# UVA-Computer-Vision-Lab/FrameINO

Hardware: AMD Instinct MI355X
Metric: denoise-steps/sec (Wan2.2-5B FrameINO, 49f 704x1280, cond+uncond DiT forward + CFG + Euler) (higher is better)
Workload: dtype bf16; 1 GPU; wan2.2-5b-49f-704x1280; layers=30, id_frames=1, hip_graph=False, parallelism=single, dead_rows_last_block=1760

## Files before the change

### frameino_amd/csrc/fino_elementwise.hip

```cpp
#include <type_traits>

#include "fino_common.h"
#include "fino_gemm_common.h"

namespace {

constexpr int kWavesPerBlock = 4;
constexpr int kMaxPasses = 8;

template <typename T, int NP>
struct RowRegs {
    float v[NP][8];
};

#ifndef FINO_EW_NT
#define FINO_EW_NT 0
#endif
#define EW_STORE_NT(PTR_, VAL_)                                                                \
    {                                                                                          \
        const uint4 v__ = (VAL_);                                                              \
        __builtin_nontemporal_store(u32x4_t{v__.x, v__.y, v__.z, v__.w}, reinterpret_cast<u32x4_t*>(PTR_)); \
    }
#define EW_STORE(PTR_, VAL_) (*reinterpret_cast<uint4*>(PTR_) = (VAL_))

template <typename T, int NP, bool NT = false>
__device__ __forceinline__ void load_row(const uint16_t* __restrict__ p, int dim, int lane, float (&v)[NP][8]) {
#pragma unroll
    for (int i = 0; i < NP; ++i) {
        const int c = (i * 64 + lane) * 8;
        if (c < dim) {
            uint4 u;
            if constexpr (NT) {
                const u32x4_t t4 = __builtin_nontemporal_load(reinterpret_cast<const u32x4_t*>(p + c));
                u = make_uint4(t4[0], t4[1], t4[2], t4[3]);
            } else {
                u = *reinterpret_cast<const uint4*>(p + c);
            }
            unpack8<T>(u, v[i]);
        } else {
#pragma unroll
            for (int j = 0; j < 8; ++j) v[i][j] = 0.f;
        }
    }
}

template <int NP>
__device__ __forceinline__ void ln_stats(const float (&v)[NP][8], int dim, int lane, float eps, float& mean,
                                         float& rstd) {
    float s = 0.f;
#pragma unroll
    for (int i = 0; i < NP; ++i)
#pragma unroll
        for (int j = 0; j < 8; ++j) s += v[i][j];
    mean = wave_sum(s) / (float)dim;
    float q = 0.f;
#pragma unroll
    for (int i = 0; i < NP; ++i) {
        const int c = (i * 64 + lane) * 8;
        if (c < dim) {
#pragma unroll
            for (int j = 0; j < 8; ++j) {
                const float d = v[i][j] - mean;
                q += d * d;
            }
        }
    }
    const float var = wave_sum(q) / (float)dim;
    rstd = 1.0f / sqrtf(var + eps);
}

template <typename T, int NP, int MODE, bool QOUT = false>
__global__ __launch_bounds__(kWavesPerBlock * 64) void ln_modulate_kernel(
    const uint16_t* __restrict__ x, uint16_t* __restrict__ y, int64_t rows, int dim, int64_t ldx, int64_t ldy,
    const float* __restrict__ p_w, const float* __restrict__ p_b, const float* __restrict__ p_shift,
    const float* __restrict__ p_scale, int64_t mod_stride, const int32_t* __restrict__ sel, float eps,
    uint8_t* __restrict__ q = nullptr, uint8_t* __restrict__ qs = nullptr, int64_t rows_pad = 0) {
    const int lane = threadIdx.x & 63;
    const int64_t row = (int64_t)blockIdx.x * kWavesPerBlock + (threadIdx.x >> 6);
    if (row >= rows) return;
    float v[NP][8];
    load_row<T, NP, (FINO_EW_NT & 1) != 0>(x + row * ldx, dim, lane, v);
    float mean, rstd;
    ln_stats<NP>(v, dim, lane, eps, mean, rstd);
    const int64_t moff = (MODE != 1 && sel) ? (int64_t)sel[row] * mod_stride : 0;
    auto ld8 = [](const float* p, float (&o)[8]) {
        const float4 a0 = *reinterpret_cast<const float4*>(p);
        const float4 a1 = *reinterpret_cast<const float4*>(p + 4);
        o[0] = a0.x; o[1] = a0.y; o[2] = a0.z; o[3] = a0.w; o[4] = a1.x; o[5] = a1.y; o[6] = a1.z; o[7] = a1.w;
    };
#pragma unroll
    for (int i = 0; i < NP; ++i) {
        const int c = (i * 64 + lane) * 8;
        if (c >= dim) continue;
        float o[8], w[8], b[8], sc[8], sh[8];
        if (MODE != 0 && p_w) ld8(p_w + c, w);
        if (MODE != 0 && p_b) ld8(p_b + c, b);
        if (MODE != 1) { ld8(p_scale + moff + c, sc); ld8(p_shift + moff + c, sh); }
#pragma unroll
        for (int j = 0; j < 8; ++j) {
            const float n = (v[i][j] - mean) * rstd;
            if (MODE == 0) {
                o[j] = n * (1.0f + sc[j]) + sh[j];
            } else {
                float t = n;
                if (p_w) t = t * w[j];
                if (p_b) t = t + b[j];
                if (MODE == 2) t = round_to<T>(round_to<T>(t) * round_to<T>(1.0f + sc[j])) + sh[j];
                o[j] = t;
            }
        }
        if constexpr (QOUT) {
            float r8[8];
#pragma unroll
            for (int j = 0; j < 8; ++j) r8[j] = round_to<T>(o[j]);
            int e;
            const uint2 qv = fino_gemm_ns::mx_quant8(r8, e);
            *reinterpret_cast<uint2*>(q + row * dim + c) = qv;
            if ((c & 31) == 0) qs[fino_gemm_ns::mx_scale_index(row, c, rows_pad)] = (uint8_t)(e + 127);
        } else if constexpr ((FINO_EW_NT & 2) != 0) EW_STORE_NT(y + row * ldy + c, pack8<T>(o))
        else EW_STORE(y + row * ldy + c, pack8<T>(o));
    }
}

template <typename T>
__global__ __launch_bounds__(256) void gated_residual_kernel(const uint16_t* __restrict__ x,
                                                             const uint16_t* __restrict__ y,
                                                             uint16_t* __restrict__ out, int64_t rows, int dim,
                                                             int64_t ldx, int64_t ldy, int64_t ldo,
                                                             const float* __restrict__ gate, int64_t mod_stride,
                                                             const int32_t* __restrict__ sel, int staged) {
    const int chunks = dim >> 3;
    const int64_t total = rows * chunks;
    for (int64_t i = (int64_t)blockIdx.x * blockDim.x + threadIdx.x; i < total;
         i += (int64_t)gridDim.x * blockDim.x) {
        const int64_t row = i / chunks;
        const int c = (int)(i - row * chunks) * 8;
        float a[8], b[8], o[8];
        unpack8<T>(*reinterpret_cast<const uint4*>(x + row * ldx + c), a);
        unpack8<T>(*reinterpret_cast<const uint4*>(y + row * ldy + c), b);
        if (gate) {
            const float* g = gate + (sel ? (int64_t)sel[row] * mod_stride : 0) + c;
            const float4 g0 = *reinterpret_cast<const float4*>(g);
            const float4 g1 = *reinterpret_cast<const float4*>(g + 4);
            const float gg[8] = {g0.x, g0.y, g0.z, g0.w, g1.x, g1.y, g1.z, g1.w};
#pragma unroll
            for (int j = 0; j < 8; ++j) o[j] = a[j] + (staged ? round_to<T>(b[j] * gg[j]) : b[j] * gg[j]);
        } else {
#pragma unroll
            for (int j = 0; j < 8; ++j) o[j] = a[j] + b[j];
        }
        *reinterpret_cast<uint4*>(out + row * ldo + c) = pack8<T>(o);
    }
}

template <typename T, int NP>
__device__ __forceinline__ void rmsnorm_rope_row(uint16_t* __restrict__ xrow, int64_t row, int dim,
                                                 const uint16_t* __restrict__ w, float eps,
                                                 const float* __restrict__ cos_t, const float* __restrict__ sin_t,
                                                 int head_dim, float out_scale, uint16_t* __restrict__ out,
                                                 const int64_t* __restrict__ head_off,
                                                 const int64_t* __restrict__ head_ld, int lane) {
    float v[NP][8];
    load_row<T, NP>(xrow, dim, lane, v);
    float rs = 1.f;
    if (w) {
        float q = 0.f;
#pragma unroll
        for (int i = 0; i < NP; ++i)
#pragma unroll
            for (int j = 0; j < 8; ++j) q += v[i][j] * v[i][j];
        const float var = wave_sum(q) / (float)dim;
        rs = 1.0f / sqrtf(var + eps);
    }
    const int half = head_dim >> 1;
#pragma unroll
    for (int i = 0; i < NP; ++i) {
        const int c = (i * 64 + lane) * 8;
        if (c >= dim) continue;
        float o[8];
        if (w) {
            float ww[8];
            unpack8<T>(*reinterpret_cast<const uint4*>(w + c), ww);
#pragma unroll
            for (int j = 0; j < 8; ++j) o[j] = round_to<T>(round_to<T>(v[i][j] * rs) * ww[j]);
        } else {
#pragma unroll
            for (int j = 0; j < 8; ++j) o[j] = v[i][j];
        }
        if (cos_t) {
            const int pidx = (c % head_dim) >> 1;
            const float4 cs = *reinterpret_cast<const float4*>(cos_t + row * half + pidx);
            const float4 sn = *reinterpret_cast<const float4*>(sin_t + row * half + pidx);
            const float cc[4] = {cs.x, cs.y, cs.z, cs.w};
            const float ss[4] = {sn.x, sn.y, sn.z, sn.w};
#pragma unroll
            for (int j = 0; j < 4; ++j) {
                const float x1 = o[2 * j], x2 = o[2 * j + 1];
                o[2 * j] = x1 * cc[j] - x2 * ss[j];
                o[2 * j + 1] = x1 * ss[j] + x2 * cc[j];
            }
        }
#pragma unroll
        for (int j = 0; j < 8; ++j) o[j] *= out_scale;
        if (out) {
            const int hd = c / head_dim;
            EW_STORE(out + head_off[hd] + row * head_ld[hd] + (c - hd * head_dim), pack8<T>(o));
        } else {
            EW_STORE(xrow + c, pack8<T>(o));
        }
    }
}

struct RmsRopeParts {
    const uint16_t* w[3];
    float eps[3];
    float out_scale[3];
    int rope[3];
};
template <typename T, int NP>
__global__ __launch_bounds__(kWavesPerBlock * 64) void rmsnorm_rope_kernel(uint16_t* __restrict__ x, int64_t rows,
                                                                           int dim, int64_t ldx, const RmsRopeParts pp,
                                                                           const float* __restrict__ cos_t,
                                                                           const float* __restrict__ sin_t,
                                                                           int head_dim, uint16_t* __restrict__ out,
                                                                           const int64_t* __restrict__ head_off,
                                                                           const int64_t* __restrict__ head_ld) {
    const int lane = threadIdx.x & 63;
    const int64_t row = (int64_t)blockIdx.x * kWavesPerBlock + (threadIdx.x >> 6);
    if (row >= rows) return;
    const int s = blockIdx.y;
    const bool rope = pp.rope[s] != 0;
    rmsnorm_rope_row<T, NP>(x + row * ldx + (int64_t)s * dim, row, dim, pp.w[s], pp.eps[s], rope ? cos_t : nullptr,
                            rope ? sin_t : nullptr, head_dim, pp.out_scale[s], out,
                            head_off ? head_off + (int64_t)s * (dim / head_dim) : nullptr, head_ld, lane);
}

template <typename T, int NP>
__global__ __launch_bounds__(kWavesPerBlock * 64) void row_rrms_kernel(const uint16_t* __restrict__ x, int64_t rows, int dim,
                                                                       int64_t ldx, float eps, float* __restrict__ rrms) {
    const int lane = threadIdx.x & 63;
    const int64_t row = (int64_t)blockIdx.x * kWavesPerBlock + (threadIdx.x >> 6);
    if (row >= rows) return;
    float v[NP][8];
    load_row<T, NP>(x + row * ldx, dim, lane, v);
    float q = 0.f;
#pragma unroll
    for (int i = 0; i < NP; ++i)
#pragma unroll
        for (int j = 0; j < 8; ++j) q += v[i][j] * v[i][j];
    const float var = wave_sum(q) / (float)dim;
    if (lane == 0) rrms[row] = 1.0f / sqrtf(var + eps);
}

template <typename T>
__global__ __launch_bounds__(256) void headnorm_rope_kernel(uint16_t* __restrict__ x, int batch, int64_t rows,
                                                            int heads, int head_dim, int64_t ldx,
                                                            int64_t batch_stride, const uint16_t* __restrict__ w,
                                                            const uint16_t* __restrict__ b, float eps,
                                                            const float* __restrict__ cos_t,
                                                            const float* __restrict__ sin_t, int64_t rope_row0,
                                                            float out_scale) {
    const int lanes_per_head = head_dim >> 3;
    const int64_t chunks_per_row = (int64_t)heads * lanes_per_head;
    const int64_t total = (int64_t)batch * rows * chunks_per_row;
    const int64_t i = (int64_t)blockIdx.x * blockDim.x + threadIdx.x;
    const bool active = i < total;
    const int64_t ii = active ? i : total - 1;
    const int64_t br = ii / chunks_per_row;
    const int cw = (int)(ii - br * chunks_per_row);
    const int64_t bi = br / rows;
    const int64_t row = br - bi * rows;
    const int cin = (cw % lanes_per_head) * 8;
    uint16_t* p = x + bi * batch_stride + row * ldx + (int64_t)cw * 8;
    float v[8];
    unpack8<T>(*reinterpret_cast<const uint4*>(p), v);
    if (w) {
        float s = 0.f;
#pragma unroll
        for (int j = 0; j < 8; ++j) s += v[j];
        for (int off = lanes_per_head >> 1; off > 0; off >>= 1) s += __shfl_xor(s, off, 64);
        const float mean = s / (float)head_dim;
        float q = 0.f;
#pragma unroll
        for (int j = 0; j < 8; ++j) {
            const float d = v[j] - mean;
            q += d * d;
        }
        for (int off = lanes_per_head >> 1; off > 0; off >>= 1) q += __shfl_xor(q, off, 64);
        const float rstd = 1.0f / sqrtf(q / (float)head_dim + eps);
        float ww[8], bb[8];
        unpack8<T>(*reinterpret_cast<const uint4*>(w + cin), ww);
        unpack8<T>(*reinterpret_cast<const uint4*>(b + cin), bb);
#pragma unroll
        for (int j = 0; j < 8; ++j) v[j] = round_to<T>((v[j] - mean) * rstd * ww[j] + bb[j]);
    }
    if (cos_t && row >= rope_row0) {
        const float* cp = cos_t + (row - rope_row0) * head_dim + cin;
        const float* sp = sin_t + (row - rope_row0) * head_dim + cin;
        float cc[8], ss[8];
        *reinterpret_cast<float4*>(cc) = *reinterpret_cast<const float4*>(cp);
        *reinterpret_cast<float4*>(cc + 4) = *reinterpret_cast<const float4*>(cp + 4);
        *reinterpret_cast<float4*>(ss) = *reinterpret_cast<const float4*>(sp);
        *reinterpret_cast<float4*>(ss + 4) = *reinterpret_cast<const float4*>(sp + 4);
        float o[8];
#pragma unroll
        for (int j = 0; j < 4; ++j) {
            const float xr = v[2 * j], xi = v[2 * j + 1];
            o[2 * j] = xr * cc[2 * j] + (-xi) * ss[2 * j];
            o[2 * j + 1] = xi * cc[2 * j + 1] + xr * ss[2 * j + 1];
        }
#pragma unroll
        for (int j = 0; j < 8; ++j) v[j] = o[j];
    }
#pragma unroll
    for (int j = 0; j < 8; ++j) v[j] *= out_scale;
    if (active) *reinterpret_cast<uint4*>(p) = pack8<T>(v);
}
// ... 120 lines not shown
    const float sa = coef[0], sb = coef[1], m1 = coef[2], m2 = coef[3], m3 = coef[4], m4 = coef[5], mn = coef[6];
    const float g = coef[7];
    const bool use_old = coef[8] != 0.f;
    for (int64_t i = (int64_t)blockIdx.x * blockDim.x + threadIdx.x; i < n_lat; i += (int64_t)gridDim.x * blockDim.x) {
        float v;
        if (has_uncond) {
            const float u = T::to_f32(pred[i]);
            const float c = T::to_f32(pred[batch_stride + i]);
            v = u + g * (c - u);
        } else {
            v = T::to_f32(pred[i]);
        }
        const float x = T::to_f32(lat[i]);
        const float x0 = round_to<T>(sa * x) - sb * v;
        const float d = use_old ? m3 * x0 - m4 * x0_old[i] : x0;
        const float nz = round_to<T>(mn * T::to_f32(noise[i]));
        lat[i] = T::from_f32(round_to<T>(m1 * x) - m2 * d + nz);
        x0_old[i] = x0;
    }
}

template <typename T>
__device__ __forceinline__ float round_product(float a, float b) {
    if constexpr (std::is_same<T, F16>::value) {
        uint32_t r = 0;
        asm("v_fma_mixlo_f16 %0, %1, %2, 0" : "+v"(r) : "v"(a), "v"(b));
        return F16::to_f32((uint16_t)r);
    } else {
        return round_to<T>(a * b);
    }
}

template <typename T>
__global__ __launch_bounds__(256) void cfg_unipc_kernel(const uint16_t* __restrict__ pc, const uint16_t* __restrict__ pu,
                                                        float* __restrict__ x, float* __restrict__ last,
                                                        float* __restrict__ m0, float* __restrict__ m1, int C, int Fg,
                                                        int Ft, int HW, const float* __restrict__ coef) {
    const float g = coef[0], sigma = coef[1], use_corr = coef[2];
    const float Cx = coef[3], C0 = coef[4], C1 = coef[5], Ct = coef[6], Px = coef[7], P0 = coef[8], P1 = coef[9];
    const int64_t total = (int64_t)C * Fg * HW;
    for (int64_t i = (int64_t)blockIdx.x * blockDim.x + threadIdx.x; i < total;
         i += (int64_t)gridDim.x * blockDim.x) {
        const int s = (int)(i % HW);
        const int f = (int)((i / HW) % Fg);
        const int c = (int)(i / ((int64_t)HW * Fg));
        const int64_t pi = ((int64_t)c * Ft + f) * HW + s;
        float v = T::to_f32(pc[pi]);
        if (pu) {
            const float u = T::to_f32(pu[pi]);
            v = round_to<T>(u + round_to<T>(g * round_to<T>(v - u)));
        }
        const float xv = x[i], a0 = m0[i];
        const float mt = xv - round_product<T>(sigma, v);
        const float xc = use_corr != 0.f ? Cx * last[i] + C0 * a0 + C1 * m1[i] + Ct * mt : xv;
        x[i] = Px * xc + P0 * mt + P1 * a0;
        last[i] = xc;
        m1[i] = a0;
        m0[i] = mt;
    }
}

template <int NPmax, typename F>
inline bool dispatch_np(int dim, F&& f) {
    const int np = (dim + 511) / 512;
    switch (np) {
        case 1: f(std::integral_constant<int, 1>{}); return true;
        case 2: f(std::integral_constant<int, 2>{}); return true;
        case 3: f(std::integral_constant<int, 3>{}); return true;
        case 4: f(std::integral_constant<int, 4>{}); return true;
        case 5: f(std::integral_constant<int, 5>{}); return true;
        case 6: f(std::integral_constant<int, 6>{}); return true;
        case 7: f(std::integral_constant<int, 7>{}); return true;
        case 8: f(std::integral_constant<int, 8>{}); return true;
        default: return false;
    }
}

inline int grid_1d(int64_t total, int block = 256) {
    int64_t g = (total + block - 1) / block;
    const int64_t cap = 256 * 8;
    return (int)(g < 1 ? 1 : (g > cap ? cap : g));
}

template <int MODE>
int launch_ln_q(const void* x, void* q, void* qs, int64_t rows, int dim, int64_t ldx, const float* w, const float* b,
                const float* shift, const float* scale, int64_t mod_stride, const int32_t* sel, float eps, int dtype,
                hipStream_t st) {
    const dim3 grid((unsigned)((rows + kWavesPerBlock - 1) / kWavesPerBlock)), block(kWavesPerBlock * 64);
    const int64_t rows_pad = (rows + 255) / 256 * 256;
    const bool ok = dispatch_np<kMaxPasses>(dim, [&](auto np) {
        constexpr int NP = decltype(np)::value;
        if (dtype == FINO_BF16)
            ln_modulate_kernel<BF16, NP, MODE, true><<<grid, block, 0, st>>>((const uint16_t*)x, nullptr, rows, dim, ldx, 0, w,
                                                                           b, shift, scale, mod_stride, sel, eps,
                                                                           (uint8_t*)q, (uint8_t*)qs, rows_pad);
        else
            ln_modulate_kernel<F16, NP, MODE, true><<<grid, block, 0, st>>>((const uint16_t*)x, nullptr, rows, dim, ldx, 0, w,
                                                                          b, shift, scale, mod_stride, sel, eps,
                                                                          (uint8_t*)q, (uint8_t*)qs, rows_pad);
    });
    FINO_CHECK(ok, FINO_ERR_UNSUPPORTED, "layernorm: dim %d > %d unsupported", dim, kMaxPasses * 512);
    FINO_LAUNCH_CHECK();
    return FINO_OK;
}

template <int MODE>
int launch_ln(const void* x, void* y, int64_t rows, int dim, int64_t ldx, int64_t ldy, const float* w, const float* b,
              const float* shift, const float* scale, int64_t mod_stride, const int32_t* sel, float eps, int dtype,
              hipStream_t st) {
    const dim3 grid((unsigned)((rows + kWavesPerBlock - 1) / kWavesPerBlock)), block(kWavesPerBlock * 64);
    const bool ok = dispatch_np<kMaxPasses>(dim, [&](auto np) {
        constexpr int NP = decltype(np)::value;
        if (dtype == FINO_BF16)
            ln_modulate_kernel<BF16, NP, MODE><<<grid, block, 0, st>>>((const uint16_t*)x, (uint16_t*)y, rows, dim,
                                                                     ldx, ldy, w, b, shift, scale, mod_stride, sel, eps);
        else
            ln_modulate_kernel<F16, NP, MODE><<<grid, block, 0, st>>>((const uint16_t*)x, (uint16_t*)y, rows, dim,
                                                                    ldx, ldy, w, b, shift, scale, mod_stride, sel, eps);
    });
    FINO_CHECK(ok, FINO_ERR_UNSUPPORTED, "layernorm: dim %d > %d unsupported", dim, kMaxPasses * 512);
    FINO_LAUNCH_CHECK();
    return FINO_OK;
}

}

#define CHECK_ROWS_DIM(fn)                                                                                    \
    FINO_CHECK(dtype == FINO_BF16 || dtype == FINO_F16, FINO_ERR_ARG, fn ": dtype %d", dtype);                \
    FINO_CHECK(rows >= 0 && dim > 0 && dim % 8 == 0, FINO_ERR_ARG, fn ": rows=%lld dim=%d (dim %% 8 != 0)",   \
               (long long)rows, dim);                                                                         \
    if (rows == 0) return FINO_OK;

extern "C" int fino_adaln_modulate(const void* x, void* y, int64_t rows, int dim, int64_t ldx, int64_t ldy,
                                   const float* shift, const float* scale, int64_t mod_stride, const int32_t* sel,
                                   float eps, int dtype, void* stream) {
    CHECK_ROWS_DIM("fino_adaln_modulate");
    FINO_CHECK(x && y && shift && scale, FINO_ERR_ARG, "fino_adaln_modulate: null pointer");
    FINO_CHECK(ldx % 8 == 0 && ldy % 8 == 0 && mod_stride % 4 == 0 && fino_aligned16(x) && fino_aligned16(y) &&
                   fino_aligned16(shift) && fino_aligned16(scale),
               FINO_ERR_ARG, "fino_adaln_modulate: 16-byte alignment required");
    return launch_ln<0>(x, y, rows, dim, ldx, ldy, nullptr, nullptr, shift, scale, mod_stride, sel, eps, dtype,
                        (hipStream_t)stream);
}

extern "C" int fino_ln_mxfp8(int mode, const void* x, void* q, void* scales, int64_t rows, int dim, int64_t ldx,
                             const float* w, const float* b, const float* shift, const float* scale, int64_t mod_stride,
                             const int32_t* sel, float eps, int dtype, void* stream) {
    CHECK_ROWS_DIM("fino_ln_mxfp8");
    FINO_CHECK(mode >= 0 && mode <= 2 && x && q && scales, FINO_ERR_ARG, "fino_ln_mxfp8: mode %d / null pointer", mode);
    FINO_CHECK(mode == 1 || (shift && scale), FINO_ERR_ARG, "fino_ln_mxfp8: modulation rows missing");
    FINO_CHECK(dim % 128 == 0, FINO_ERR_ARG, "fino_ln_mxfp8: dim=%d must be a multiple of 128", dim);
    FINO_CHECK(ldx % 8 == 0 && mod_stride % 4 == 0 && fino_aligned16(x) && fino_aligned16(shift) && fino_aligned16(scale) &&
                   fino_aligned16(w) && fino_aligned16(b) && ((uintptr_t)q & 7) == 0,
               FINO_ERR_ARG, "fino_ln_mxfp8: alignment");
    hipStream_t st = (hipStream_t)stream;
    if (mode == 0) return launch_ln_q<0>(x, q, scales, rows, dim, ldx, nullptr, nullptr, shift, scale, mod_stride, sel, eps, dtype, st);
    if (mode == 1) return launch_ln_q<1>(x, q, scales, rows, dim, ldx, w, b, nullptr, nullptr, 0, nullptr, eps, dtype, st);
    return launch_ln_q<2>(x, q, scales, rows, dim, ldx, w, b, shift, scale, mod_stride, sel, eps, dtype, st);
}

extern "C" int fino_layernorm(const void* x, void* y, int64_t rows, int dim, int64_t ldx, int64_t ldy,
                              const float* w, const float* b, float eps, int dtype, void* stream) {
    CHECK_ROWS_DIM("fino_layernorm");
    FINO_CHECK(x && y, FINO_ERR_ARG, "fino_layernorm: null pointer");
    FINO_CHECK(ldx % 8 == 0 && ldy % 8 == 0 && fino_aligned16(x) && fino_aligned16(y) && fino_aligned16(w) &&
                   fino_aligned16(b),
               FINO_ERR_ARG, "fino_layernorm: 16-byte alignment required");
    return launch_ln<1>(x, y, rows, dim, ldx, ldy, w, b, nullptr, nullptr, 0, nullptr, eps, dtype, (hipStream_t)stream);
}

extern "C" int fino_layernorm_zero(const void* x, void* y, int64_t rows, int dim, int64_t ldx, int64_t ldy,
                                   const float* w, const float* b, const float* shift, const float* scale,
                                   int64_t mod_stride, const int32_t* sel, float eps, int dtype, void* stream) {
    CHECK_ROWS_DIM("fino_layernorm_zero");
    FINO_CHECK(x && y && shift && scale, FINO_ERR_ARG, "fino_layernorm_zero: null pointer");
    FINO_CHECK(ldx % 8 == 0 && ldy % 8 == 0 && mod_stride % 4 == 0 && fino_aligned16(x) && fino_aligned16(y) &&
                   fino_aligned16(shift) && fino_aligned16(scale) && fino_aligned16(w) && fino_aligned16(b),
               FINO_ERR_ARG, "fino_layernorm_zero: 16-byte alignment required");
    return launch_ln<2>(x, y, rows, dim, ldx, ldy, w, b, shift, scale, mod_stride, sel, eps, dtype, (hipStream_t)stream);
}

static int gated_residual_impl(const void* x, const void* y, void* out, int64_t rows, int dim, int64_t ldx, int64_t ldy,
                               int64_t ldo, const float* gate, int64_t mod_stride, const int32_t* sel, int staged,
                               int dtype, void* stream);

extern "C" int fino_gated_residual(const void* x, const void* y, void* out, int64_t rows, int dim, int64_t ldx,
                                   int64_t ldy, int64_t ldo, const float* gate, int64_t mod_stride,
                                   const int32_t* sel, int dtype, void* stream) {
    return gated_residual_impl(x, y, out, rows, dim, ldx, ldy, ldo, gate, mod_stride, sel, 0, dtype, stream);
}

extern "C" int fino_gated_residual_staged(const void* x, const void* y, void* out, int64_t rows, int dim, int64_t ldx,
                                          int64_t ldy, int64_t ldo, const float* gate, int64_t mod_stride,
                                          const int32_t* sel, int dtype, void* stream) {
    return gated_residual_impl(x, y, out, rows, dim, ldx, ldy, ldo, gate, mod_stride, sel, 1, dtype, stream);
}

static int gated_residual_impl(const void* x, const void* y, void* out, int64_t rows, int dim, int64_t ldx, int64_t ldy,
                               int64_t ldo, const float* gate, int64_t mod_stride, const int32_t* sel, int staged,
                               int dtype, void* stream) {
    CHECK_ROWS_DIM("fino_gated_residual");
    FINO_CHECK(x && y && out, FINO_ERR_ARG, "fino_gated_residual: null pointer");
    FINO_CHECK(ldx % 8 == 0 && ldy % 8 == 0 && ldo % 8 == 0 && mod_stride % 4 == 0 && fino_aligned16(x) &&
                   fino_aligned16(y) && fino_aligned16(out) && fino_aligned16(gate),
               FINO_ERR_ARG, "fino_gated_residual: 16-byte alignment required");
    const int grid = grid_1d(rows * (dim / 8));
    hipStream_t st = (hipStream_t)stream;
    if (dtype == FINO_BF16)
        gated_residual_kernel<BF16><<<grid, 256, 0, st>>>((const uint16_t*)x, (const uint16_t*)y, (uint16_t*)out,
                                                          rows, dim, ldx, ldy, ldo, gate, mod_stride, sel, staged);
    else
        gated_residual_kernel<F16><<<grid, 256, 0, st>>>((const uint16_t*)x, (const uint16_t*)y, (uint16_t*)out,
                                                         rows, dim, ldx, ldy, ldo, gate, mod_stride, sel, staged);
    FINO_LAUNCH_CHECK();
    return FINO_OK;
}

static int rmsnorm_rope_impl(void* x, int64_t rows, int dim, int64_t ldx, int parts, const RmsRopeParts& pp,
                             const float* cos_t, const float* sin_t, int head_dim, void* out, const int64_t* head_off,
                             const int64_t* head_ld, int dtype, void* stream) {
    CHECK_ROWS_DIM("fino_rmsnorm_rope");
    FINO_CHECK(x, FINO_ERR_ARG, "fino_rmsnorm_rope: null pointer");
    FINO_CHECK(parts >= 1 && parts <= 3, FINO_ERR_ARG, "fino_rmsnorm_rope: parts %d", parts);
    bool any_rope = false;
    for (int i = 0; i < parts; ++i) {
        FINO_CHECK(pp.out_scale[i] > 0.f, FINO_ERR_ARG, "fino_rmsnorm_rope_scaled: out_scale must be > 0");
        FINO_CHECK(fino_aligned16(pp.w[i]), FINO_ERR_ARG, "fino_rmsnorm_rope: 16-byte alignment required");
        any_rope = any_rope || pp.rope[i];
    }
    FINO_CHECK((cos_t == nullptr) == (sin_t == nullptr), FINO_ERR_ARG, "fino_rmsnorm_rope: cos/sin must both be set");
    FINO_CHECK(!any_rope || cos_t, FINO_ERR_ARG, "fino_rmsnorm_rope: a segment asks for RoPE without tables");
    FINO_CHECK((!cos_t && !out) || (head_dim > 0 && head_dim % 8 == 0 && dim % head_dim == 0), FINO_ERR_ARG,
               "fino_rmsnorm_rope: head_dim=%d must divide dim=%d and be a multiple of 8", head_dim, dim);
    FINO_CHECK(ldx % 8 == 0 && fino_aligned16(x) && fino_aligned16(cos_t) && fino_aligned16(sin_t) && fino_aligned16(out),
               FINO_ERR_ARG, "fino_rmsnorm_rope: 16-byte alignment required");
    FINO_CHECK(parts == 1 || dim % 8 == 0, FINO_ERR_ARG, "fino_rmsnorm_rope: segments need dim % 8 == 0");
    const dim3 grid((unsigned)((rows + kWavesPerBlock - 1) / kWavesPerBlock), (unsigned)parts), block(kWavesPerBlock * 64);
    hipStream_t st = (hipStream_t)stream;
    const bool ok = dispatch_np<kMaxPasses>(dim, [&](auto np) {
        constexpr int NP = decltype(np)::value;
        if (dtype == FINO_BF16)
            rmsnorm_rope_kernel<BF16, NP><<<grid, block, 0, st>>>((uint16_t*)x, rows, dim, ldx, pp, cos_t, sin_t, head_dim,
                                                                  (uint16_t*)out, head_off, head_ld);
        else
            rmsnorm_rope_kernel<F16, NP><<<grid, block, 0, st>>>((uint16_t*)x, rows, dim, ldx, pp, cos_t, sin_t, head_dim,
                                                                 (uint16_t*)out, head_off, head_ld);
    });
    FINO_CHECK(ok, FINO_ERR_UNSUPPORTED, "fino_rmsnorm_rope: dim %d > %d unsupported", dim, kMaxPasses * 512);
    FINO_LAUNCH_CHECK();
    return FINO_OK;
}

extern "C" int fino_row_rrms(const void* x, int64_t rows, int dim, int64_t ldx, float eps, float* rrms, int dtype, void* stream) {
    FINO_CHECK(dtype == FINO_BF16 || dtype == FINO_F16, FINO_ERR_ARG, "fino_row_rrms: dtype %d", dtype);
    FINO_CHECK(x && rrms && rows >= 0 && dim > 0 && dim % 8 == 0 && ldx % 8 == 0 && fino_aligned16(x), FINO_ERR_ARG,
               "fino_row_rrms: bad arguments");
    if (rows == 0) return FINO_OK;
    const dim3 grid((unsigned)((rows + kWavesPerBlock - 1) / kWavesPerBlock)), block(kWavesPerBlock * 64);
    hipStream_t st = (hipStream_t)stream;
    const bool ok = dispatch_np<kMaxPasses>(dim, [&](auto np) {
        constexpr int NP = decltype(np)::value;
        if (dtype == FINO_BF16) row_rrms_kernel<BF16, NP><<<grid, block, 0, st>>>((const uint16_t*)x, rows, dim, ldx, eps, rrms);
        else row_rrms_kernel<F16, NP><<<grid, block, 0, st>>>((const uint16_t*)x, rows, dim, ldx, eps, rrms);
    });
    FINO_CHECK(ok, FINO_ERR_UNSUPPORTED, "fino_row_rrms: dim %d > %d unsupported", dim, kMaxPasses * 512);
    FINO_LAUNCH_CHECK();
    return FINO_OK;
}

static RmsRopeParts one_part(const void* weight, float eps, float out_scale, bool rope) {
    RmsRopeParts pp = {};
    pp.w[0] = (const uint16_t*)weight; pp.eps[0] = eps; pp.out_scale[0] = out_scale; pp.rope[0] = rope ? 1 : 0;
    return pp;
}

extern "C" int fino_rmsnorm_rope_scaled(void* x, int64_t rows, int dim, int64_t ldx, const void* weight, float eps,
                                        const float* cos_t, const float* sin_t, int head_dim, float out_scale, int dtype,
                                        void* stream) {
    return rmsnorm_rope_impl(x, rows, dim, ldx, 1, one_part(weight, eps, out_scale, cos_t != nullptr), cos_t, sin_t,
                             head_dim, nullptr, nullptr, nullptr, dtype, stream);
}

extern "C" int fino_rmsnorm_rope_scatter(const void* x, int64_t rows, int dim, int64_t ldx, const void* weight, float eps,
                                         const float* cos_t, const float* sin_t, int head_dim, float out_scale, void* out,
                                         const int64_t* head_off, const int64_t* head_ld, int dtype, void* stream) {
    FINO_CHECK(out && head_off && head_ld, FINO_ERR_ARG, "fino_rmsnorm_rope_scatter: null destination / table");
    return rmsnorm_rope_impl(const_cast<void*>(x), rows, dim, ldx, 1, one_part(weight, eps, out_scale, cos_t != nullptr),
                             cos_t, sin_t, head_dim, out, head_off, head_ld, dtype, stream);
}

extern "C" int fino_qkv_rmsnorm_rope(void* qkv, int64_t rows, int dim, int64_t ldx, const void* q_weight, float q_eps,
                                     const void* k_weight, float k_eps, const float* cos_t, const float* sin_t,
                                     int head_dim, float q_out_scale, void* out, const int64_t* head_off,
                                     const int64_t* head_ld, int dtype, void* stream) {
    FINO_CHECK((out == nullptr) == (head_off == nullptr) && (out == nullptr) == (head_ld == nullptr), FINO_ERR_ARG,
               "fino_qkv_rmsnorm_rope: out, head_off and head_ld go together");
    RmsRopeParts pp = {};
    pp.w[0] = (const uint16_t*)q_weight; pp.eps[0] = q_eps; pp.out_scale[0] = q_out_scale; pp.rope[0] = cos_t ? 1 : 0;
    pp.w[1] = (const uint16_t*)k_weight; pp.eps[1] = k_eps; pp.out_scale[1] = 1.0f; pp.rope[1] = cos_t ? 1 : 0;
    pp.w[2] = nullptr; pp.eps[2] = 0.f; pp.out_scale[2] = 1.0f; pp.rope[2] = 0;
    return rmsnorm_rope_impl(qkv, rows, dim, ldx, out ? 3 : 2, pp, cos_t, sin_t, head_dim, out, head_off, head_ld, dtype,
                             stream);
}

extern "C" int fino_rmsnorm_rope(void* x, int64_t rows, int dim, int64_t ldx, const void* weight, float eps,
                                 const float* cos_t, const float* sin_t, int head_dim, int dtype, void* stream) {
    return fino_rmsnorm_rope_scaled(x, rows, dim, ldx, weight, eps, cos_t, sin_t, head_dim, 1.0f, dtype, stream);
}

extern "C" int fino_headnorm_rope_scaled(void* x, int batch, int64_t rows, int heads, int head_dim, int64_t ldx,
                                         int64_t batch_stride, const void* w, const void* b, float eps,
                                         const float* cos_t, const float* sin_t, int64_t rope_row0, float out_scale,
                                         int dtype, void* stream) {
    FINO_CHECK(dtype == FINO_BF16 || dtype == FINO_F16, FINO_ERR_ARG, "fino_headnorm_rope: dtype %d", dtype);
    FINO_CHECK(x && batch >= 0 && rows >= 0 && heads > 0 && out_scale > 0.f, FINO_ERR_ARG, "fino_headnorm_rope: bad shape");
    FINO_CHECK(head_dim == 16 || head_dim == 32 || head_dim == 64 || head_dim == 128, FINO_ERR_UNSUPPORTED,
               "fino_headnorm_rope: head_dim %d not in {16,32,64,128}", head_dim);
    FINO_CHECK((w == nullptr) == (b == nullptr) && (cos_t == nullptr) == (sin_t == nullptr), FINO_ERR_ARG,
               "fino_headnorm_rope: w/b and cos/sin come in pairs");
    FINO_CHECK(ldx % 8 == 0 && batch_stride % 8 == 0 && fino_aligned16(x) && fino_aligned16(w) && fino_aligned16(b) &&
                   fino_aligned16(cos_t) && fino_aligned16(sin_t),
               FINO_ERR_ARG, "fino_headnorm_rope: 16-byte alignment required");
    const int64_t total = (int64_t)batch * rows * heads * (head_dim / 8);
    if (total == 0) return FINO_OK;
    const unsigned grid = (unsigned)((total + 255) / 256);
    hipStream_t st = (hipStream_t)stream;
    if (dtype == FINO_BF16)
        headnorm_rope_kernel<BF16><<<grid, 256, 0, st>>>((uint16_t*)x, batch, rows, heads, head_dim, ldx, batch_stride,
// ... 144 lines not shown
```

### include/frameino_hip.h

```cpp
#ifndef FRAMEINO_HIP_H
#define FRAMEINO_HIP_H
#include <stdint.h>

#ifdef __cplusplus
extern "C" {
#endif

#define FINO_VERSION 103

enum { FINO_BF16 = 0, FINO_F16 = 1, FINO_F32 = 2 };
enum {
    FINO_OK = 0,
    FINO_ERR_ARG = -1,
    FINO_ERR_LAUNCH = -2,
    FINO_ERR_UNSUPPORTED = -3
};

int fino_version(void);
const char* fino_last_error(void);

enum { FINO_TUNE_GEMM_GROUP_M = 0, FINO_TUNE_GEMM_RASTER = 1, FINO_TUNE_CONV_LOOP = 2, FINO_TUNE_GEMM_TILE_M = 3,
       FINO_TUNE_ATTN_KERNEL = 4, FINO_TUNE_ATTN_FP8_KERNEL = 5, FINO_TUNE_ATTN_WALK_GRID = 6, FINO_TUNE_COUNT = 8 };
int fino_tune_set(int key, int value);
int fino_tune_get(int key);

int fino_adaln_modulate(const void* x, void* y, int64_t rows, int dim, int64_t ldx, int64_t ldy,
                        const float* shift, const float* scale, int64_t mod_stride, const int32_t* sel,
                        float eps, int dtype, void* stream);

int fino_layernorm(const void* x, void* y, int64_t rows, int dim, int64_t ldx, int64_t ldy, const float* w,
                   const float* b, float eps, int dtype, void* stream);

int fino_gated_residual(const void* x, const void* y, void* out, int64_t rows, int dim, int64_t ldx, int64_t ldy,
                        int64_t ldo, const float* gate, int64_t mod_stride, const int32_t* sel, int dtype,
                        void* stream);

int fino_gated_residual_staged(const void* x, const void* y, void* out, int64_t rows, int dim, int64_t ldx, int64_t ldy,
                               int64_t ldo, const float* gate, int64_t mod_stride, const int32_t* sel, int dtype,
                               void* stream);

int fino_layernorm_zero(const void* x, void* y, int64_t rows, int dim, int64_t ldx, int64_t ldy, const float* w,
                        const float* b, const float* shift, const float* scale, int64_t mod_stride, const int32_t* sel,
                        float eps, int dtype, void* stream);

int fino_ln_mxfp8(int mode, const void* x, void* q, void* scales, int64_t rows, int dim, int64_t ldx, const float* w,
                  const float* b, const float* shift, const float* scale, int64_t mod_stride, const int32_t* sel,
                  float eps, int dtype, void* stream);

int fino_rmsnorm_rope(void* x, int64_t rows, int dim, int64_t ldx, const void* weight, float eps,
                      const float* cos_t, const float* sin_t, int head_dim, int dtype, void* stream);
int fino_rmsnorm_rope_scaled(void* x, int64_t rows, int dim, int64_t ldx, const void* weight, float eps,
                             const float* cos_t, const float* sin_t, int head_dim, float out_scale, int dtype,
                             void* stream);

int fino_rmsnorm_rope_scatter(const void* x, int64_t rows, int dim, int64_t ldx, const void* weight, float eps,
                              const float* cos_t, const float* sin_t, int head_dim, float out_scale, void* out,
                              const int64_t* head_off, const int64_t* head_ld, int dtype, void* stream);

int fino_qkv_rmsnorm_rope(void* qkv, int64_t rows, int dim, int64_t ldx, const void* q_weight, float q_eps,
                          const void* k_weight, float k_eps, const float* cos_t, const float* sin_t, int head_dim,
                          float q_out_scale, void* out, const int64_t* head_off, const int64_t* head_ld, int dtype,
                          void* stream);

int fino_headnorm_rope(void* x, int batch, int64_t rows, int heads, int head_dim, int64_t ldx, int64_t batch_stride,
                       const void* w, const void* b, float eps, const float* cos_t, const float* sin_t,
                       int64_t rope_row0, int dtype, void* stream);
int fino_headnorm_rope_scaled(void* x, int batch, int64_t rows, int heads, int head_dim, int64_t ldx,
                              int64_t batch_stride, const void* w, const void* b, float eps, const float* cos_t,
                              const float* sin_t, int64_t rope_row0, float out_scale, int dtype, void* stream);

#define FINO_ATTN_SCALE_FOLDED (-1.0f)
int fino_attn_fwd(const void* q, const void* k, const void* v, void* o, int batch, int heads, int64_t lq,
                  int64_t lk, int head_dim, int64_t q_bs, int64_t q_rs, int64_t q_hs, int64_t k_bs, int64_t k_rs,
                  int64_t k_hs, int64_t v_bs, int64_t v_rs, int64_t v_hs, int64_t o_bs, int64_t o_rs,
                  int64_t o_hs, float scale, int dtype, void* stream);
enum { FINO_FP8_P_EXP2 = 0, FINO_FP8_P_RAMP = 1 };
int64_t fino_attn_fp8_kv_bytes(int batch, int heads, int64_t lk, int head_dim);
int fino_attn_fwd_fp8(const void* q, const void* k, const void* v, void* o, int batch, int heads, int64_t lq, int64_t lk,
                      int head_dim, int64_t q_bs, int64_t q_rs, int64_t k_bs, int64_t k_rs, int64_t v_bs, int64_t v_rs,
                      int64_t o_bs, int64_t o_rs, float scale, int dtype, int p_mode, void* kv_workspace,
                      int64_t kv_workspace_bytes, void* stream);
int64_t fino_attn_fp8_smooth_kv_bytes(int batch, int heads, int64_t lk, int head_dim);
int fino_attn_fwd_fp8_smooth(const void* q, const void* k, const void* v, void* o, int batch, int heads, int64_t lq, int64_t lk,
                             int head_dim, int64_t q_bs, int64_t q_rs, int64_t k_bs, int64_t k_rs, int64_t v_bs, int64_t v_rs,
                             int64_t o_bs, int64_t o_rs, float scale, int dtype, int p_mode, void* kv_workspace,
                             int64_t kv_workspace_bytes, void* stream);

int fino_attn_tail_supported(int batch, int heads, int64_t lq, int64_t lk, int head_dim);
int fino_attn_fwd_tail(const void* q, const void* k, const void* v, void* o, int batch, int heads, int64_t lq, int64_t lk,
                       int head_dim, int64_t q_bs, int64_t q_rs, int64_t q_hs, int64_t k_bs, int64_t k_rs, int64_t k_hs,
                       int64_t v_bs, int64_t v_rs, int64_t v_hs, int64_t o_bs, int64_t o_rs, int64_t o_hs, float scale,
                       int dtype, const int* lk_b, const float* tail_mult, void* stream);

int fino_attn_ranges_supported(int batch, int heads, int64_t lq, int64_t lk, int head_dim);
int fino_attn_fwd_ranges(const void* q, const void* k, const void* v, void* o, int batch, int heads, int64_t lq, int64_t lk,
                         int head_dim, int64_t q_bs, int64_t q_rs, int64_t q_hs, int64_t k_bs, int64_t k_rs, int64_t k_hs,
                         int64_t v_bs, int64_t v_rs, int64_t v_hs, int64_t o_bs, int64_t o_rs, int64_t o_hs, float scale,
                         int dtype, const int* ranges, void* stream);

int fino_attn_probs_supported(int batch, int heads, int64_t lq, int64_t lk, int head_dim);
int fino_attn_probs(const void* q, const void* k, void* p, int batch, int heads, int64_t lq, int64_t lk, int head_dim,
                    int64_t q_bs, int64_t q_rs, int64_t q_hs, int64_t k_bs, int64_t k_rs, int64_t k_hs, int kp, int64_t p_bs,
                    int64_t p_rs, float scale, int dtype, const int* lk_b, const float* tail_mult, const float* q_rrms,
                    int64_t q_rrms_bs, const void* q_weight, void* stream);
int fino_row_rrms(const void* x, int64_t rows, int dim, int64_t ldx, float eps, float* rrms, int dtype, void* stream);
// ... 148 lines not shown
```

Before: 3.838 denoise-steps/s.

## Make rmsnorm_rope kernel persistent with next-row prefetch via buffer loads

Converts the fused RMSNorm+RoPE kernel into a grid-stride persistent kernel whose grid is sized from occupancy and CU count. While normalising the current row it prefetches the next row into registers using buffer loads with bounds-sized resources. It also double-buffers the per-pass weight and cos/sin table loads, with sched barriers fixing the instruction order. This aims to hide global memory latency in a bandwidth-bound kernel, at the cost of extra register pressure and a new tune knob for the grid size.

```diff
diff --git a/frameino_amd/csrc/fino_elementwise.hip b/frameino_amd/csrc/fino_elementwise.hip
--- a/frameino_amd/csrc/fino_elementwise.hip
+++ b/frameino_amd/csrc/fino_elementwise.hip
@@ -22,6 +22,48 @@
         __builtin_nontemporal_store(u32x4_t{v__.x, v__.y, v__.z, v__.w}, reinterpret_cast<u32x4_t*>(PTR_)); \
     }
 #define EW_STORE(PTR_, VAL_) (*reinterpret_cast<uint4*>(PTR_) = (VAL_))
+#define EW_PASS_FENCE() __builtin_amdgcn_sched_barrier(0)
+#define EW_PASS_LIVE(I_, C_) ((I_) < NP - 1 || (C_) < dim)
+
+__device__ __forceinline__ __amdgpu_buffer_rsrc_t ew_rsrc(const void* p, int bytes) {
+    return __builtin_amdgcn_make_buffer_rsrc(const_cast<void*>(p), 0, bytes, 0x00020000);
+}
+__device__ __forceinline__ uint4 ew_ld16(__amdgpu_buffer_rsrc_t r, int byte_off) {
+    const u32x4_t t = __builtin_amdgcn_raw_buffer_load_b128(r, byte_off, 0, 0);
+    return make_uint4(t[0], t[1], t[2], t[3]);
+}
+
+template <int NP>
+__device__ __forceinline__ void load_row_raw(const uint16_t* p, int dim, bool live, int lane, uint4 (&u)[NP]) {
+    const __amdgpu_buffer_rsrc_t r = ew_rsrc(p, live ? dim * 2 : 0);
+#pragma unroll
+    for (int i = 0; i < NP; ++i) u[i] = ew_ld16(r, (i * 64 + lane) * 16);
+}
+
+template <int NP>
+__device__ __forceinline__ void ew_forget(uint4 (&u)[NP]) {
+#pragma unroll
+    for (int i = 0; i < NP; ++i) asm volatile("" : "+v"(u[i].x), "+v"(u[i].y), "+v"(u[i].z), "+v"(u[i].w));
+}
+
+__device__ __forceinline__ int64_t first_row() {
+    return (int64_t)blockIdx.x * kWavesPerBlock + __builtin_amdgcn_readfirstlane((int)(threadIdx.x >> 6));
+}
+__device__ __forceinline__ int64_t row_stride() { return (int64_t)gridDim.x * kWavesPerBlock; }
+
+template <typename T, int NP>
+__device__ __forceinline__ float row_sumsq(const uint4 (&u)[NP]) {
+    float q = 0.f;
+#pragma unroll
+    for (int i = 0; i < NP; ++i) {
+        float f[8];
+        unpack8<T>(u[i], f);
+#pragma unroll
+        for (int j = 0; j < 8; ++j) q += f[j] * f[j];
+    }
+    return q;
+}
+
 
 template <typename T, int NP, bool NT = false>
 __device__ __forceinline__ void load_row(const uint16_t* __restrict__ p, int dim, int lane, float (&v)[NP][8]) {
@@ -154,61 +196,77 @@
 }
 
 template <typename T, int NP>
-__device__ __forceinline__ void rmsnorm_rope_row(uint16_t* __restrict__ xrow, int64_t row, int dim,
+__device__ __forceinline__ void rmsnorm_rope_row(uint4 (&u)[NP], const uint16_t* xnext, bool more, uint16_t* xrow, int64_t row,
+                                                 int dim,
                                                  const uint16_t* __restrict__ w, float eps,
                                                  const float* __restrict__ cos_t, const float* __restrict__ sin_t,
                                                  int head_dim, float out_scale, uint16_t* __restrict__ out,
                                                  const int64_t* __restrict__ head_off,
                                                  const int64_t* __restrict__ head_ld, int lane) {
-    float v[NP][8];
-    load_row<T, NP>(xrow, dim, lane, v);
+    const int half = head_dim >> 1;
+    struct Tabs { uint4 w, cs, sn; };
+    const __amdgpu_buffer_rsrc_t r_w = ew_rsrc(w, w ? dim * 2 : 0);
+    const __amdgpu_buffer_rsrc_t r_cs = ew_rsrc(cos_t ? cos_t + row * half : nullptr, cos_t ? half * 4 : 0);
+    const __amdgpu_buffer_rsrc_t r_sn = ew_rsrc(cos_t ? sin_t + row * half : nullptr, cos_t ? half * 4 : 0);
+    auto load_tabs = [&](int i, Tabs& t) {
+        const int c = (i * 64 + lane) * 8;
+        t.w = ew_ld16(r_w, c * 2);
+        const int pidx = cos_t ? (c % head_dim) >> 1 : 0;
+        t.cs = ew_ld16(r_cs, pidx * 4);
+        t.sn = ew_ld16(r_sn, pidx * 4);
+    };
+    Tabs t;
+    load_tabs(0, t);
+    uint4 un[NP];
+    load_row_raw<NP>(xnext, dim, more, lane, un);
+    EW_PASS_FENCE();
     float rs = 1.f;
     if (w) {
-        float q = 0.f;
-#pragma unroll
-        for (int i = 0; i < NP; ++i)
-#pragma unroll
-            for (int j = 0; j < 8; ++j) q += v[i][j] * v[i][j];
-        const float var = wave_sum(q) / (float)dim;
+        const float var = wave_sum(row_sumsq<T, NP>(u)) / (float)dim;
         rs = 1.0f / sqrtf(var + eps);
-    }
-    const int half = head_dim >> 1;
+        ew_forget(u);
+    }
 #pragma unroll
     for (int i = 0; i < NP; ++i) {
         const int c = (i * 64 + lane) * 8;
-        if (c >= dim) continue;
-        float o[8];
-        if (w) {
-            float ww[8];
-            unpack8<T>(*reinterpret_cast<const uint4*>(w + c), ww);
-#pragma unroll
-            for (int j = 0; j < 8; ++j) o[j] = round_to<T>(round_to<T>(v[i][j] * rs) * ww[j]);
-        } else {
-#pragma unroll
-            for (int j = 0; j < 8; ++j) o[j] = v[i][j];
-        }
-        if (cos_t) {
-            const int pidx = (c % head_dim) >> 1;
-            const float4 cs = *reinterpret_cast<const float4*>(cos_t + row * half + pidx);
-            const float4 sn = *reinterpret_cast<const float4*>(sin_t + row * half + pidx);
-            const float cc[4] = {cs.x, cs.y, cs.z, cs.w};
-            const float ss[4] = {sn.x, sn.y, sn.z, sn.w};
-#pragma unroll
-            for (int j = 0; j < 4; ++j) {
-                const float x1 = o[2 * j], x2 = o[2 * j + 1];
-                o[2 * j] = x1 * cc[j] - x2 * ss[j];
-                o[2 * j + 1] = x1 * ss[j] + x2 * cc[j];
+        Tabs tn;
+        if (i + 1 < NP) load_tabs(i + 1, tn);
+        EW_PASS_FENCE();
+        if (EW_PASS_LIVE(i, c)) {
+            float v[8], o[8];
+            unpack8<T>(u[i], v);
+            if (w) {
+                float ww[8];
+                unpack8<T>(t.w, ww);
+#pragma unroll
+                for (int j = 0; j < 8; ++j) o[j] = round_to<T>(round_to<T>(v[j] * rs) * ww[j]);
+            } else {
+#pragma unroll
+                for (int j = 0; j < 8; ++j) o[j] = v[j];
             }
-        }
-#pragma unroll
-        for (int j = 0; j < 8; ++j) o[j] *= out_scale;
-        if (out) {
-            const int hd = c / head_dim;
-            EW_STORE(out + head_off[hd] + row * head_ld[hd] + (c - hd * head_dim), pack8<T>(o));
-        } else {
-            EW_STORE(xrow + c, pack8<T>(o));
-        }
-    }
+            if (cos_t) {
+                const float cc[4] = {__uint_as_float(t.cs.x), __uint_as_float(t.cs.y), __uint_as_float(t.cs.z), __uint_as_float(t.cs.w)};
+                const float ss[4] = {__uint_as_float(t.sn.x), __uint_as_float(t.sn.y), __uint_as_float(t.sn.z), __uint_as_float(t.sn.w)};
+#pragma unroll
+                for (int j = 0; j < 4; ++j) {
+                    const float x1 = o[2 * j], x2 = o[2 * j + 1];
+                    o[2 * j] = x1 * cc[j] - x2 * ss[j];
+                    o[2 * j + 1] = x1 * ss[j] + x2 * cc[j];
+                }
+            }
+#pragma unroll
+            for (int j = 0; j < 8; ++j) o[j] *= out_scale;
+            if (out) {
+                const int hd = c / head_dim;
+                EW_STORE(out + head_off[hd] + row * head_ld[hd] + (c - hd * head_dim), pack8<T>(o));
+            } else {
+                EW_STORE(xrow + c, pack8<T>(o));
+            }
+        }
+        EW_PASS_FENCE();
+        t = tn;
+    }
+    for (int i = 0; i < NP; ++i) u[i] = un[i];
 }
 
 struct RmsRopeParts {
@@ -218,21 +276,31 @@
     int rope[3];
 };
 template <typename T, int NP>
-__global__ __launch_bounds__(kWavesPerBlock * 64) void rmsnorm_rope_kernel(uint16_t* __restrict__ x, int64_t rows,
-                                                                           int dim, int64_t ldx, const RmsRopeParts pp,
+__global__ __launch_bounds__(kWavesPerBlock * 64) void rmsnorm_rope_kernel(uint16_t* x, int64_t rows, int dim, int64_t ldx,
+                                                                           const RmsRopeParts pp,
                                                                            const float* __restrict__ cos_t,
                                                                            const float* __restrict__ sin_t,
                                                                            int head_dim, uint16_t* __restrict__ out,
                                                                            const int64_t* __restrict__ head_off,
                                                                            const int64_t* __restrict__ head_ld) {
     const int lane = threadIdx.x & 63;
-    const int64_t row = (int64_t)blockIdx.x * kWavesPerBlock + (threadIdx.x >> 6);
+    const int64_t stride = row_stride();
+    int64_t row = first_row();
     if (row >= rows) return;
     const int s = blockIdx.y;
     const bool rope = pp.rope[s] != 0;
-    rmsnorm_rope_row<T, NP>(x + row * ldx + (int64_t)s * dim, row, dim, pp.w[s], pp.eps[s], rope ? cos_t : nullptr,
-                            rope ? sin_t : nullptr, head_dim, pp.out_scale[s], out,
-                            head_off ? head_off + (int64_t)s * (dim / head_dim) : nullptr, head_ld, lane);
+    uint16_t* xs = x + (int64_t)s * dim;
+    uint4 u[NP];
+    load_row_raw<NP>(xs + row * ldx, dim, true, lane, u);
+    for (;;) {
+        const int64_t next = row + stride;
+        const bool more = next < rows;
+        rmsnorm_rope_row<T, NP>(u, xs + (more ? next : row) * ldx, more, xs + row * ldx, row, dim, pp.w[s], pp.eps[s], rope ? cos_t : nullptr,
+                                rope ? sin_t : nullptr, head_dim, pp.out_scale[s], out,
+                                head_off ? head_off + (int64_t)s * (dim / head_dim) : nullptr, head_ld, lane);
+        if (!more) break;
+        row = next;
+    }
 }
 
 template <typename T, int NP>
@@ -519,6 +587,29 @@
     return (int)(g < 1 ? 1 : (g > cap ? cap : g));
 }
 
+template <auto Kernel>
+inline unsigned row_grid(int64_t rows, int split = 1) {
+    const int64_t want = (rows + kWavesPerBlock - 1) / kWavesPerBlock;
+    const int forced = fino_tune_get(FINO_TUNE_EW_GRID);
+    if (forced > 0) return (unsigned)(forced < want ? forced : want);
+    static std::atomic<int> resident[kFinoMaxDevices];
+    const int dev = fino_current_device();
+    int r = resident[dev].load(std::memory_order_relaxed);
+    if (r == 0) {
+        int per_cu = 0, cus = 0;
+        if (hipOccupancyMaxActiveBlocksPerMultiprocessor(&per_cu, Kernel, kWavesPerBlock * 64, 0) != hipSuccess || per_cu < 1)
+            per_cu = 4;
+        if (hipDeviceGetAttribute(&cus, hipDeviceAttributeMultiprocessorCount, dev) != hipSuccess || cus < 1) cus = 256;
+        r = per_cu * cus;
+        resident[dev].store(r, std::memory_order_relaxed);
+    }
+    int64_t cap = r / (split > 1 ? split : 1);
+    if (cap < 1) cap = 1;
+    if (want <= cap) return (unsigned)want;
+    const int64_t rounds = (want + cap - 1) / cap;
+    return (unsigned)((want + rounds - 1) / rounds);
+}
+
 template <int MODE>
 int launch_ln_q(const void* x, void* q, void* qs, int64_t rows, int dim, int64_t ldx, const float* w, const float* b,
                 const float* shift, const float* scale, int64_t mod_stride, const int32_t* sel, float eps, int dtype,
@@ -672,15 +763,15 @@
     FINO_CHECK(ldx % 8 == 0 && fino_aligned16(x) && fino_aligned16(cos_t) && fino_aligned16(sin_t) && fino_aligned16(out),
                FINO_ERR_ARG, "fino_rmsnorm_rope: 16-byte alignment required");
     FINO_CHECK(parts == 1 || dim % 8 == 0, FINO_ERR_ARG, "fino_rmsnorm_rope: segments need dim % 8 == 0");
-    const dim3 grid((unsigned)((rows + kWavesPerBlock - 1) / kWavesPerBlock), (unsigned)parts), block(kWavesPerBlock * 64);
+    const dim3 block(kWavesPerBlock * 64);
     hipStream_t st = (hipStream_t)stream;
     const bool ok = dispatch_np<kMaxPasses>(dim, [&](auto np) {
         constexpr int NP = decltype(np)::value;
         if (dtype == FINO_BF16)
-            rmsnorm_rope_kernel<BF16, NP><<<grid, block, 0, st>>>((uint16_t*)x, rows, dim, ldx, pp, cos_t, sin_t, head_dim,
+            rmsnorm_rope_kernel<BF16, NP><<<dim3(row_grid<rmsnorm_rope_kernel<BF16, NP>>(rows, parts), (unsigned)parts), block, 0, st>>>((uint16_t*)x, rows, dim, ldx, pp, cos_t, sin_t, head_dim,
                                                                   (uint16_t*)out, head_off, head_ld);
         else
-            rmsnorm_rope_kernel<F16, NP><<<grid, block, 0, st>>>((uint16_t*)x, rows, dim, ldx, pp, cos_t, sin_t, head_dim,
+            rmsnorm_rope_kernel<F16, NP><<<dim3(row_grid<rmsnorm_rope_kernel<F16, NP>>(rows, parts), (unsigned)parts), block, 0, st>>>((uint16_t*)x, rows, dim, ldx, pp, cos_t, sin_t, head_dim,
                                                                  (uint16_t*)out, head_off, head_ld);
     });
     FINO_CHECK(ok, FINO_ERR_UNSUPPORTED, "fino_rmsnorm_rope: dim %d > %d unsupported", dim, kMaxPasses * 512);
diff --git a/include/frameino_hip.h b/include/frameino_hip.h
--- a/include/frameino_hip.h
+++ b/include/frameino_hip.h
@@ -20,7 +20,8 @@
 const char* fino_last_error(void);
 
 enum { FINO_TUNE_GEMM_GROUP_M = 0, FINO_TUNE_GEMM_RASTER = 1, FINO_TUNE_CONV_LOOP = 2, FINO_TUNE_GEMM_TILE_M = 3,
-       FINO_TUNE_ATTN_KERNEL = 4, FINO_TUNE_ATTN_FP8_KERNEL = 5, FINO_TUNE_ATTN_WALK_GRID = 6, FINO_TUNE_COUNT = 8 };
+       FINO_TUNE_ATTN_KERNEL = 4, FINO_TUNE_ATTN_FP8_KERNEL = 5, FINO_TUNE_ATTN_WALK_GRID = 6, FINO_TUNE_EW_GRID = 7,
+       FINO_TUNE_COUNT = 8 };
 int fino_tune_set(int key, int value);
 int fino_tune_get(int key);
 
```

Measured after the change: 3.849 denoise-steps/s, median of 6. About the same (+0.3%).
